# danini/multi-h

Hardware: AMD Instinct MI355X
Metric: scored homography hypotheses/sec (50k pts x 100k models) (higher is better)
Workload: dtype f64

## Files before the change

multi-h_amd/csrc/dlt4.hip:

```cpp

#include "mh_kernels.hpp"
#include "mh_device.hpp"

namespace mh {

__device__ __forceinline__ unsigned long long splitmix64(unsigned long long z)
{
    z += 0x9E3779B97F4A7C15ull;
    z = (z ^ (z >> 30)) * 0xBF58476D1CE4E5B9ull;
    z = (z ^ (z >> 27)) * 0x94D049BB133111EBull;
    return z ^ (z >> 31);
}

template <int K, int MAXDRAW>
__device__ __forceinline__ void sample_tuple(unsigned long long seed, unsigned long long m,
                                             unsigned int N, int* out)
{
    int got = 0;
    for (unsigned int c = 0; c < MAXDRAW && got < K; ++c) {
        const unsigned long long r = splitmix64(seed + (m << 8) + c);
        const int idx = (int)(((r >> 32) * (unsigned long long)N) >> 32);
        bool dup = false;
        for (int k = 0; k < got; ++k) dup = dup || (out[k] == idx);
        if (!dup) out[got++] = idx;
    }
    for (; got < K; ++got) out[got] = out[0];
}

__device__ __forceinline__ void sample4(unsigned long long seed, unsigned long long m,
                                        unsigned int N, int out[4])
{
    sample_tuple<4, 64>(seed, m, N, out);
}

constexpr int DLT_SAMPLER_UNIFORM = 0, DLT_SAMPLER_LOCAL = 1;

__device__ __forceinline__ void sample4_by(unsigned long long seed, unsigned long long c, unsigned int N, int out[4])
{
    sample4(seed, c, N, out);
}

__device__ __forceinline__ void sample4_by(unsigned long long seed, unsigned long long c, unsigned int N, int out[4],
                                           const int* __restrict__ nbr, int k, int uniform_per_16)
{
    if ((int)(c & 15ull) < uniform_per_16) { sample4(seed, c, N, out); return; }
    const unsigned long long base = seed + (c << 8);
    const int i0 = (int)(((splitmix64(base) >> 32) * (unsigned long long)N) >> 32);
    const int* __restrict__ row = nbr + (size_t)i0 * (size_t)k;
    int o1 = -1, o2 = -1, o3 = -1, got = 1;
    for (unsigned int j = 1; j < 64 && got < 4; ++j) {
        const unsigned long long r = splitmix64(base + j);
        const int cand = row[(int)(((r >> 32) * (unsigned long long)(unsigned int)k) >> 32)];
        if (cand != i0 && cand != o1 && cand != o2) {
            o1 = got == 1 ? cand : o1;
            o2 = got == 2 ? cand : o2;
            o3 = got == 3 ? cand : o3;
            ++got;
        }
    }
    out[0] = i0;
    out[1] = got > 1 ? o1 : i0;
    out[2] = got > 2 ? o2 : i0;
    out[3] = got > 3 ? o3 : i0;
}

__device__ __forceinline__ void rr_pair(int r, int slot, int& p, int& q)
{
    const int k = slot + 1;
    const int a = (r + k) % 9, b = (r + 9 - k) % 9;
    p = a < b ? a : b;
    q = a < b ? b : a;
}

constexpr int HPW = 16;
constexpr int WROWS = 17, WCOLS = 9;

__device__ __forceinline__ void wave_sync()
{
#ifdef MH_DLT_WAVE_FENCES
    __builtin_amdgcn_fence(__ATOMIC_RELEASE, "wavefront");
    __builtin_amdgcn_wave_barrier();
    __builtin_amdgcn_fence(__ATOMIC_ACQUIRE, "wavefront");
#else
    asm volatile("" ::: "memory");
    __builtin_amdgcn_wave_barrier();
    asm volatile("" ::: "memory");
#endif
}

__device__ __forceinline__ void null9_sweeps(double (*W)[HPW], int hs, int slot, bool live)
{
#define WE(r, c) W[(r) * WCOLS + (c)][hs]
    for (int sweep = 0; sweep < 30; ++sweep) {
        int rotated = 0;
        for (int r = 0; r < 9; ++r) {
            int p, q;
            rr_pair(r, slot, p, q);
            double alpha = 0.0, beta = 0.0, gamma = 0.0;
#pragma unroll
            for (int i = 0; i < 8; ++i) {
                const double wp = WE(i, p), wq = WE(i, q);
                alpha = alpha + wp * wp;
                beta = beta + wq * wq;
                gamma = gamma + wp * wq;
            }
            const bool rot = live && (gamma != 0.0) && (gamma * gamma > 1e-30 * (alpha * beta)) &&
                             (alpha >= 1e-28) && (beta >= 1e-28);
            if (rot) {
                ++rotated;
                const double zeta = (beta - alpha) / (2.0 * gamma);
                const double sg = (zeta >= 0.0) ? 1.0 : -1.0;
                const double t = sg / (fabs(zeta) + sqrt(1.0 + zeta * zeta));
                const double c = 1.0 / sqrt(1.0 + t * t);
                const double s = c * t;
#pragma unroll
                for (int i = 0; i < WROWS; ++i) {
                    const double wp = WE(i, p), wq = WE(i, q);
                    WE(i, p) = c * wp - s * wq;
                    WE(i, q) = s * wp + c * wq;
                }
            }
            wave_sync();
        }
        if (!__any(rotated)) break;
    }
#undef WE
}

__device__ __forceinline__ void null9_vector(double (*W)[HPW], int hs, double g[9])
{
#define WE(r, c) W[(r) * WCOLS + (c)][hs]
    int jm = 0;
    double best = 0.0;
    for (int j = 0; j < 9; ++j) {
        double a = 0.0;
        for (int i = 0; i < 8; ++i) a = a + WE(i, j) * WE(i, j);
        if (j == 0 || a < best) { best = a; jm = j; }
    }
    for (int j = 0; j < 9; ++j) g[j] = WE(8 + j, jm);
#undef WE
}

template <int SAMPLER, class... TABLE>
__global__ void __launch_bounds__(256) __attribute__((amdgpu_num_vgpr(72)))
k_dlt4_lds(const double* __restrict__ x1, const double* __restrict__ y1,
       const double* __restrict__ x2, const double* __restrict__ y2, int N,
       unsigned long long seed, long long first, int M, int* __restrict__ idx_out,
       double* __restrict__ H_out, TABLE... table)
{
    static_assert(sizeof...(TABLE) == (SAMPLER == DLT_SAMPLER_LOCAL ? 3 : 0), "the local sampler takes nbr, k, uniform_per_16");
    __builtin_amdgcn_s_setprio(3);
    __shared__ double sW[4][WROWS * WCOLS][HPW];
    const int lane = threadIdx.x & 63;
    const int wave = threadIdx.x >> 6;
    const int hs = lane & (HPW - 1);
    const int slot = lane >> 4;
    const int m = (blockIdx.x * 4 + wave) * HPW + hs;
    const bool live = m < M;
    double (*W)[HPW] = sW[wave];
#define WE(r, c) W[(r) * WCOLS + (c)][hs]

    int id[4] = { 0, 0, 0, 0 };
    double sx[4], sy[4], dx[4], dy[4];
    if (live) sample4_by(seed, (unsigned long long)(first + m), (unsigned int)N, id, table...);
#pragma unroll
    for (int k = 0; k < 4; ++k) {
        sx[k] = x1[id[k]]; sy[k] = y1[id[k]]; dx[k] = x2[id[k]]; dy[k] = y2[id[k]];
    }
    if (live && slot == 0 && idx_out) {
#pragma unroll
        for (int k = 0; k < 4; ++k) idx_out[4 * (size_t)m + k] = id[k];
    }
    double cx1 = ((sx[0] + sx[1]) + sx[2]) + sx[3], cy1 = ((sy[0] + sy[1]) + sy[2]) + sy[3];
    double cx2 = ((dx[0] + dx[1]) + dx[2]) + dx[3], cy2 = ((dy[0] + dy[1]) + dy[2]) + dy[3];
    cx1 = cx1 * 0.25; cy1 = cy1 * 0.25; cx2 = cx2 * 0.25; cy2 = cy2 * 0.25;
    double d1 = 0.0, d2 = 0.0;
#pragma unroll
    for (int k = 0; k < 4; ++k) {
        const double ax = sx[k] - cx1, ay = sy[k] - cy1, bx = dx[k] - cx2, by = dy[k] - cy2;
        d1 = d1 + sqrt(ax * ax + ay * ay);
        d2 = d2 + sqrt(bx * bx + by * by);
    }
    const double s1 = sqrt(2.0) / (d1 * 0.25), s2 = sqrt(2.0) / (d2 * 0.25);

    {
        double x = 0.0, y = 0.0, u = 0.0, v = 0.0;
#pragma unroll
        for (int k = 0; k < 4; ++k)
            if (k == slot) {
                x = (sx[k] - cx1) * s1; y = (sy[k] - cy1) * s1;
                u = (dx[k] - cx2) * s2; v = (dy[k] - cy2) * s2;
            }
        const int r0 = 2 * slot, r1 = 2 * slot + 1;
        WE(r0, 0) = -x; WE(r0, 1) = -y; WE(r0, 2) = -1.0; WE(r0, 3) = 0.0; WE(r0, 4) = 0.0;
        WE(r0, 5) = 0.0; WE(r0, 6) = u * x; WE(r0, 7) = u * y; WE(r0, 8) = u;
        WE(r1, 0) = 0.0; WE(r1, 1) = 0.0; WE(r1, 2) = 0.0; WE(r1, 3) = -x; WE(r1, 4) = -y;
        WE(r1, 5) = -1.0; WE(r1, 6) = v * x; WE(r1, 7) = v * y; WE(r1, 8) = v;
        if (slot < 3)
            for (int i = 3 * slot; i < 3 * slot + 3; ++i)
                for (int j = 0; j < 9; ++j) WE(8 + i, j) = (i == j) ? 1.0 : 0.0;
    }
    __syncthreads();

    null9_sweeps(W, hs, slot, live);

    if (live && slot == 0) {
        double g[9];
        null9_vector(W, hs, g);
        double A1[9];
#pragma unroll
        for (int r = 0; r < 3; ++r) {
            const double a = g[3 * r], b = g[3 * r + 1], c = g[3 * r + 2];
            A1[3 * r] = a * s1;
            A1[3 * r + 1] = b * s1;
            A1[3 * r + 2] = (c - (a * s1) * cx1) - (b * s1) * cy1;
        }
        const double is2 = 1.0 / s2;
        double Hh[9];
#pragma unroll
        for (int j = 0; j < 3; ++j) {
            Hh[j] = A1[j] * is2 + cx2 * A1[6 + j];
            Hh[3 + j] = A1[3 + j] * is2 + cy2 * A1[6 + j];
            Hh[6 + j] = A1[6 + j];
        }
        double fro = 0.0;
#pragma unroll
        for (int j = 0; j < 9; ++j) fro = fro + Hh[j] * Hh[j];
        double sc = 1.0 / sqrt(fro);
        if (Hh[8] < 0.0) sc = -sc;
        double* out = H_out + 9 * (size_t)m;
#pragma unroll
        for (int j = 0; j < 9; ++j) out[j] = Hh[j] * sc;
    }
#undef WE
}

struct Col { double v[WROWS]; };

template <int CTRL, int BANK_MASK>
__device__ __forceinline__ double dpp_merge(double old, double src)
{
    const int lo = __builtin_amdgcn_update_dpp(__double2loint(old), __double2loint(src), CTRL, 0xF, BANK_MASK, false);
    const int hi = __builtin_amdgcn_update_dpp(__double2hiint(old), __double2hiint(src), CTRL, 0xF, BANK_MASK, false);
    return __hiloint2double(hi, lo);
}

__device__ __forceinline__ void shift_columns(Col& a, Col& b, Col& c)
{
#pragma unroll
    for (int i = 0; i < WROWS; ++i) {
        c.v[i] = dpp_merge<0x114 , 0xE>(c.v[i], b.v[i]);
        b.v[i] = dpp_merge<0x104 , 0x7>(b.v[i], a.v[i]);
    }
}

__device__ __forceinline__ int rotate_pair(Col& P, Col& Q, bool swapped, bool live)
{
    double alpha = 0.0, beta = 0.0, gamma = 0.0;
#pragma unroll
    for (int i = 0; i < 8; ++i) {
        const double wp = P.v[i], wq = Q.v[i];
        alpha = alpha + wp * wp;
        beta = beta + wq * wq;
        gamma = gamma + wp * wq;
    }
    const bool rot = live && (gamma != 0.0) && (gamma * gamma > 1e-30 * (alpha * beta)) &&
                     (alpha >= 1e-28) && (beta >= 1e-28);
    if (rot) {
        const double zeta = (beta - alpha) / (2.0 * gamma);
        const bool pos = swapped ? (zeta > 0.0) : (zeta >= 0.0);
        const double sg = pos ? 1.0 : -1.0;
        const double t = sg / (fabs(zeta) + sqrt(1.0 + zeta * zeta));
        const double c = 1.0 / sqrt(1.0 + t * t);
        const double s = c * t;
#pragma unroll
        for (int i = 0; i < WROWS; ++i) {
            const double wp = P.v[i], wq = Q.v[i];
            P.v[i] = c * wp - s * wq;
            Q.v[i] = s * wp + c * wq;
        }
    }
    return rot ? 1 : 0;
}

__host__ __device__ constexpr unsigned swapped_rounds(int s)
{
    unsigned m = 0;
    for (int r = 0; r < 9; ++r) {
        const int k = s + 1, a = (r + k) % 9, b = (r + 9 - k) % 9;
        if (a > b) m |= 1u << r;
    }
    return m;
}

__device__ __forceinline__ void dlt_column(int c, const double* x, const double* y, const double* u, const double* v, Col& out)
{
#pragma unroll
    for (int k = 0; k < 4; ++k) {
        const double e0[9] = { -x[k], -y[k], -1.0, 0.0, 0.0, 0.0, u[k] * x[k], u[k] * y[k], u[k] };
        const double e1[9] = { 0.0, 0.0, 0.0, -x[k], -y[k], -1.0, v[k] * x[k], v[k] * y[k], v[k] };
        double r0 = e0[0], r1 = e1[0];
#pragma unroll
        for (int j = 1; j < 9; ++j) {
            r0 = (c == j) ? e0[j] : r0;
            r1 = (c == j) ? e1[j] : r1;
        }
        out.v[2 * k] = r0;
        out.v[2 * k + 1] = r1;
    }
#pragma unroll
    for (int i = 0; i < 9; ++i) out.v[8 + i] = (i == c) ? 1.0 : 0.0;
}

__device__ __forceinline__ double column_norm(const Col& a)
{
    double n = 0.0;
#pragma unroll
    for (int i = 0; i < 8; ++i) n = n + a.v[i] * a.v[i];
    return n;
}

template <int SAMPLER, class... TABLE>
__global__ void __launch_bounds__(256)
k_dlt4(const double* __restrict__ x1, const double* __restrict__ y1,
       const double* __restrict__ x2, const double* __restrict__ y2, int N,
       unsigned long long seed, long long first, int M, int* __restrict__ idx_out,
       double* __restrict__ H_out, TABLE... table)
{
    static_assert(sizeof...(TABLE) == (SAMPLER == DLT_SAMPLER_LOCAL ? 3 : 0), "the local sampler takes nbr, k, uniform_per_16");
    __builtin_amdgcn_s_setprio(3);
    __shared__ double sN[4][9][HPW];
    __shared__ double sK[4][6][HPW];
    const int lane = threadIdx.x & 63;
    const int wave = threadIdx.x >> 6;
    const int slot = (lane >> 2) & 3;
    const int hs = (lane >> 4) * 4 + (lane & 3);
    const int m = (blockIdx.x * 4 + wave) * HPW + hs;
    const bool live = m < M;

    Col A, B, C;
    {
        int id[4] = { 0, 0, 0, 0 };
        double sx[4], sy[4], dx[4], dy[4];
        if (live) sample4_by(seed, (unsigned long long)(first + m), (unsigned int)N, id, table...);
#pragma unroll
        for (int k = 0; k < 4; ++k) {
            sx[k] = x1[id[k]]; sy[k] = y1[id[k]]; dx[k] = x2[id[k]]; dy[k] = y2[id[k]];
        }
        if (live && slot == 0 && idx_out) {
#pragma unroll
            for (int k = 0; k < 4; ++k) idx_out[4 * (size_t)m + k] = id[k];
        }
        double cx1 = ((sx[0] + sx[1]) + sx[2]) + sx[3], cy1 = ((sy[0] + sy[1]) + sy[2]) + sy[3];
        double cx2 = ((dx[0] + dx[1]) + dx[2]) + dx[3], cy2 = ((dy[0] + dy[1]) + dy[2]) + dy[3];
        cx1 = cx1 * 0.25; cy1 = cy1 * 0.25; cx2 = cx2 * 0.25; cy2 = cy2 * 0.25;
        double d1 = 0.0, d2 = 0.0;
#pragma unroll
        for (int k = 0; k < 4; ++k) {
            const double ax = sx[k] - cx1, ay = sy[k] - cy1, bx = dx[k] - cx2, by = dy[k] - cy2;
            d1 = d1 + sqrt(ax * ax + ay * ay);
            d2 = d2 + sqrt(bx * bx + by * by);
        }
        const double s1 = sqrt(2.0) / (d1 * 0.25), s2 = sqrt(2.0) / (d2 * 0.25);
        if (slot == 0) {
            sK[wave][0][hs] = s1; sK[wave][1][hs] = s2; sK[wave][2][hs] = cx1;
            sK[wave][3][hs] = cy1; sK[wave][4][hs] = cx2; sK[wave][5][hs] = cy2;
        }
        double x[4], y[4], u[4], v[4];
#pragma unroll
        for (int k = 0; k < 4; ++k) {
            x[k] = (sx[k] - cx1) * s1; y[k] = (sy[k] - cy1) * s1;
            u[k] = (dx[k] - cx2) * s2; v[k] = (dy[k] - cy2) * s2;
        }
        dlt_column(slot + 1, x, y, u, v, A);
        dlt_column(8 - slot, x, y, u, v, B);
        dlt_column(0, x, y, u, v, C);
    }

    const unsigned sw = slot == 0 ? swapped_rounds(0) : slot == 1 ? swapped_rounds(1) : slot == 2 ? swapped_rounds(2) : swapped_rounds(3);
    for (int sweep = 0; sweep < 30; ++sweep) {
        unsigned long long rotated = 0;
#pragma unroll 1
        for (int r = 0; r < 9; r += 3) {
            rotated |= __ballot(rotate_pair(A, B, (sw >> r) & 1u, live));
            shift_columns(A, B, C);
            rotated |= __ballot(rotate_pair(B, C, (sw >> (r + 1)) & 1u, live));
            shift_columns(B, C, A);
            rotated |= __ballot(rotate_pair(C, A, (sw >> (r + 2)) & 1u, live));
            shift_columns(C, A, B);
        }
        if (rotated == 0) break;
    }

    sN[wave][slot + 1][hs] = column_norm(A);
    sN[wave][8 - slot][hs] = column_norm(B);
    if (slot == 0) sN[wave][0][hs] = column_norm(C);
    wave_sync();
    int jm = 0;
    {
        double best = 0.0;
        for (int j = 0; j < 9; ++j) {
            const double a = sN[wave][j][hs];
            if (j == 0 || a < best) { best = a; jm = j; }
        }
    }
    wave_sync();
    if (jm == slot + 1) {
#pragma unroll
        for (int j = 0; j < 9; ++j) sN[wave][j][hs] = A.v[8 + j];
    } else if (jm == 8 - slot) {
#pragma unroll
        for (int j = 0; j < 9; ++j) sN[wave][j][hs] = B.v[8 + j];
    } else if (jm == 0 && slot == 0) {
#pragma unroll
        for (int j = 0; j < 9; ++j) sN[wave][j][hs] = C.v[8 + j];
    }
    wave_sync();

    if (live && slot == 0) {
        double g[9];
#pragma unroll
        for (int j = 0; j < 9; ++j) g[j] = sN[wave][j][hs];
        const double s1 = sK[wave][0][hs], s2 = sK[wave][1][hs], cx1 = sK[wave][2][hs];
        const double cy1 = sK[wave][3][hs], cx2 = sK[wave][4][hs], cy2 = sK[wave][5][hs];
        double A1[9];
#pragma unroll
        for (int r = 0; r < 3; ++r) {
            const double a = g[3 * r], b = g[3 * r + 1], c = g[3 * r + 2];
            A1[3 * r] = a * s1;
            A1[3 * r + 1] = b * s1;
            A1[3 * r + 2] = (c - (a * s1) * cx1) - (b * s1) * cy1;
        }
        const double is2 = 1.0 / s2;
        double Hh[9];
#pragma unroll
        for (int j = 0; j < 3; ++j) {
            Hh[j] = A1[j] * is2 + cx2 * A1[6 + j];
            Hh[3 + j] = A1[3 + j] * is2 + cy2 * A1[6 + j];
            Hh[6 + j] = A1[6 + j];
        }
        double fro = 0.0;
#pragma unroll
        for (int j = 0; j < 9; ++j) fro = fro + Hh[j] * Hh[j];
        double sc = 1.0 / sqrt(fro);
        if (Hh[8] < 0.0) sc = -sc;
        double* out = H_out + 9 * (size_t)m;
#pragma unroll
        for (int j = 0; j < 9; ++j) out[j] = Hh[j] * sc;
    }
}

__global__ void __launch_bounds__(256)
k_fund8(const double* __restrict__ x1, const double* __restrict__ y1,
        const double* __restrict__ x2, const double* __restrict__ y2, int N,
        unsigned long long seed, long long first, int M, int* __restrict__ idx_out,
        double* __restrict__ F_out)
{
    __shared__ double sW[4][WROWS * WCOLS][HPW];
    const int lane = threadIdx.x & 63;
    const int wave = threadIdx.x >> 6;
    const int hs = lane & (HPW - 1);
    const int slot = lane >> 4;
    const int m = (blockIdx.x * 4 + wave) * HPW + hs;
    const bool live = m < M;
    double (*W)[HPW] = sW[wave];
#define WE(r, c) W[(r) * WCOLS + (c)][hs]

    int id[8] = { 0, 0, 0, 0, 0, 0, 0, 0 };
    if (live) sample_tuple<8, 256>(seed, (unsigned long long)(first + m), (unsigned int)N, id);
    double sx[8], sy[8], dx[8], dy[8];
#pragma unroll
    for (int k = 0; k < 8; ++k) { sx[k] = x1[id[k]]; sy[k] = y1[id[k]]; dx[k] = x2[id[k]]; dy[k] = y2[id[k]]; }
    if (live && slot == 0 && idx_out) {
#pragma unroll
        for (int k = 0; k < 8; ++k) idx_out[8 * (size_t)m + k] = id[k];
    }
    double cx1 = sx[0], cy1 = sy[0], cx2 = dx[0], cy2 = dy[0];
#pragma unroll
    for (int k = 1; k < 8; ++k) { cx1 = cx1 + sx[k]; cy1 = cy1 + sy[k]; cx2 = cx2 + dx[k]; cy2 = cy2 + dy[k]; }
    cx1 = cx1 * 0.125; cy1 = cy1 * 0.125; cx2 = cx2 * 0.125; cy2 = cy2 * 0.125;
    double d1 = 0.0, d2 = 0.0;
#pragma unroll
    for (int k = 0; k < 8; ++k) {
        const double ax = sx[k] - cx1, ay = sy[k] - cy1, bx = dx[k] - cx2, by = dy[k] - cy2;
        d1 = d1 + sqrt(ax * ax + ay * ay);
        d2 = d2 + sqrt(bx * bx + by * by);
    }
    const double s1 = sqrt(2.0) / (d1 * 0.125), s2 = sqrt(2.0) / (d2 * 0.125);

#pragma unroll
    for (int k = 0; k < 8; ++k)
        if ((k >> 1) == slot) {
            const double x = (sx[k] - cx1) * s1, y = (sy[k] - cy1) * s1;
            const double u = (dx[k] - cx2) * s2, v = (dy[k] - cy2) * s2;
            WE(k, 0) = u * x; WE(k, 1) = u * y; WE(k, 2) = u;
            WE(k, 3) = v * x; WE(k, 4) = v * y; WE(k, 5) = v;
            WE(k, 6) = x; WE(k, 7) = y; WE(k, 8) = 1.0;
        }
    if (slot < 3)
        for (int i = 3 * slot; i < 3 * slot + 3; ++i)
            for (int j = 0; j < 9; ++j) WE(8 + i, j) = (i == j) ? 1.0 : 0.0;
    __syncthreads();

    null9_sweeps(W, hs, slot, live);

    if (live && slot == 0) {
        double g[9];
        null9_vector(W, hs, g);
        double Mm[9], V[9], D[3];
        for (int i = 0; i < 3; ++i)
            for (int j = 0; j < 3; ++j) {
                double a = 0.0;
                for (int k = 0; k < 3; ++k) a = a + g[3 * k + i] * g[3 * k + j];
                Mm[3 * i + j] = a;
            }
        jacobi_sym_dev(3, Mm, V, D);
        int jm = 0;
        for (int j = 1; j < 3; ++j) if (D[j] < D[jm]) jm = j;
        const double v0 = V[0 * 3 + jm], v1 = V[1 * 3 + jm], v2 = V[2 * 3 + jm];
        double Fn[9];
        for (int r = 0; r < 3; ++r) {
            const double w = (g[3 * r] * v0 + g[3 * r + 1] * v1) + g[3 * r + 2] * v2;
            Fn[3 * r] = g[3 * r] - w * v0;
            Fn[3 * r + 1] = g[3 * r + 1] - w * v1;
            Fn[3 * r + 2] = g[3 * r + 2] - w * v2;
        }
        double B[9];
        for (int r = 0; r < 3; ++r) {
            const double a = Fn[3 * r] * s1, b = Fn[3 * r + 1] * s1;
            B[3 * r] = a; B[3 * r + 1] = b;
            B[3 * r + 2] = (Fn[3 * r + 2] - a * cx1) - b * cy1;
        }
        double Fh[9];
        const double tx = s2 * cx2, ty = s2 * cy2;
        for (int j = 0; j < 3; ++j) {
            Fh[j] = s2 * B[j];
            Fh[3 + j] = s2 * B[3 + j];
            Fh[6 + j] = (B[6 + j] - tx * B[j]) - ty * B[3 + j];
        }
        double fro = 0.0;
        for (int j = 0; j < 9; ++j) fro = fro + Fh[j] * Fh[j];
        double sc = 1.0 / sqrt(fro);
        if (Fh[8] < 0.0) sc = -sc;
        double* out = F_out + 9 * (size_t)m;
        for (int j = 0; j < 9; ++j) out[j] = Fh[j] * sc;
    }
#undef WE
}

__device__ __forceinline__ double det3_rows(const double* r0, const double* r1, const double* r2)
{
    return (r0[0] * (r1[1] * r2[2] - r1[2] * r2[1]) - r0[1] * (r1[0] * r2[2] - r1[2] * r2[0])) +
           r0[2] * (r1[0] * r2[1] - r1[1] * r2[0]);
}

__device__ __forceinline__ double cubic_newton(double c0, double c1, double c2, double c3, double t)
{
    double p = ((c3 * t + c2) * t + c1) * t + c0;
    for (int it = 0; it < 4; ++it) {
        const double dp = (3.0 * c3 * t + 2.0 * c2) * t + c1;
        const double tn = t - p / dp;
        const double pn = ((c3 * tn + c2) * tn + c1) * tn + c0;
        if (!(fabs(pn) <= fabs(p)) || !(fabs(tn) < 1e300)) break;
        t = tn; p = pn;
    }
    return t;
}

struct CubicRoots { double t0, t1, t2; int n; };

__device__ __forceinline__ CubicRoots cubic_real_roots(double c0, double c1, double c2, double c3)
{
    const double qnan = __longlong_as_double(0x7ff8000000000000ll);
    const double a = c2 / c3, b = c1 / c3, c = c0 / c3;
    const double Q = (a * a - 3.0 * b) / 9.0;
    const double R = ((2.0 * a * a * a - 9.0 * a * b) + 27.0 * c) / 54.0;
    const double Q3 = Q * Q * Q;
    const double disc = R * R - Q3;
    const double a3 = a / 3.0;
    const bool usable = (fabs(a) < 1e300) && (fabs(b) < 1e300) && (fabs(c) < 1e300) && (fabs(disc) < 1e300);
    const bool three = disc < 0.0;
    const double theta = acos(R / sqrt(Q3));
    const double sq = -2.0 * sqrt(Q);
    const double two_pi = 6.283185307179586476925286766559;
    const double u0 = sq * cos(theta / 3.0) - a3;
    const double u1 = sq * cos((theta + two_pi) / 3.0) - a3;
    const double u2 = sq * cos((theta - two_pi) / 3.0) - a3;
    double A = cbrt(fabs(R) + sqrt(disc));
    if (R >= 0.0) A = -A;
    const double B = (A == 0.0) ? 0.0 : Q / A;
    const double w0 = (A + B) - a3;
    const double w1 = -0.5 * (A + B) - a3;
    const int nr = !usable ? 0 : three ? 3 : (disc == 0.0 && Q > 0.0) ? 2 : 1;
    double r0 = nr == 0 ? qnan : cubic_newton(c0, c1, c2, c3, three ? u0 : w0);
    double r1 = nr < 2 ? qnan : cubic_newton(c0, c1, c2, c3, three ? u1 : w1);
    double r2 = nr < 3 ? qnan : cubic_newton(c0, c1, c2, c3, u2);
    { const bool sw = (r1 < r0) || (r0 != r0 && r1 == r1); const double lo = sw ? r1 : r0, hi = sw ? r0 : r1; r0 = lo; r1 = hi; }
    { const bool sw = (r2 < r1) || (r1 != r1 && r2 == r2); const double lo = sw ? r2 : r1, hi = sw ? r1 : r2; r1 = lo; r2 = hi; }
    { const bool sw = (r1 < r0) || (r0 != r0 && r1 == r1); const double lo = sw ? r1 : r0, hi = sw ? r0 : r1; r0 = lo; r1 = hi; }
    return CubicRoots{ r0, r1, r2, nr };
}

__global__ void __launch_bounds__(256)
k_fund7(const double* __restrict__ x1, const double* __restrict__ y1,
        const double* __restrict__ x2, const double* __restrict__ y2, int N,
        unsigned long long seed, long long first, int M, int* __restrict__ idx_out,
        double* __restrict__ F_out, int* __restrict__ nvalid_out)
{
    __shared__ double sW[4][WROWS * WCOLS][HPW];
    const int lane = threadIdx.x & 63;
    const int wave = threadIdx.x >> 6;
    const int hs = lane & (HPW - 1);
    const int slot = lane >> 4;
    const int m = (blockIdx.x * 4 + wave) * HPW + hs;
    const bool live = m < M;
    double (*W)[HPW] = sW[wave];
#define WE(r, c) W[(r) * WCOLS + (c)][hs]

    int id[7] = { 0, 0, 0, 0, 0, 0, 0 };
    if (live) sample_tuple<7, 256>(seed, (unsigned long long)(first + m), (unsigned int)N, id);
    double sx[7], sy[7], dx[7], dy[7];
#pragma unroll
    for (int k = 0; k < 7; ++k) { sx[k] = x1[id[k]]; sy[k] = y1[id[k]]; dx[k] = x2[id[k]]; dy[k] = y2[id[k]]; }
    if (live && slot == 0 && idx_out) {
#pragma unroll
        for (int k = 0; k < 7; ++k) idx_out[7 * (size_t)m + k] = id[k];
    }
    double cx1 = sx[0], cy1 = sy[0], cx2 = dx[0], cy2 = dy[0];
#pragma unroll
    for (int k = 1; k < 7; ++k) { cx1 = cx1 + sx[k]; cy1 = cy1 + sy[k]; cx2 = cx2 + dx[k]; cy2 = cy2 + dy[k]; }
    cx1 = cx1 / 7.0; cy1 = cy1 / 7.0; cx2 = cx2 / 7.0; cy2 = cy2 / 7.0;
    double d1 = 0.0, d2 = 0.0;
#pragma unroll
    for (int k = 0; k < 7; ++k) {
        const double ax = sx[k] - cx1, ay = sy[k] - cy1, bx = dx[k] - cx2, by = dy[k] - cy2;
        d1 = d1 + sqrt(ax * ax + ay * ay);
        d2 = d2 + sqrt(bx * bx + by * by);
    }
    const double s1 = sqrt(2.0) / (d1 / 7.0), s2 = sqrt(2.0) / (d2 / 7.0);

#pragma unroll
    for (int k = 0; k < 7; ++k)
        if ((k >> 1) == slot) {
            const double x = (sx[k] - cx1) * s1, y = (sy[k] - cy1) * s1;
            const double u = (dx[k] - cx2) * s2, v = (dy[k] - cy2) * s2;
            WE(k, 0) = u * x; WE(k, 1) = u * y; WE(k, 2) = u;
            WE(k, 3) = v * x; WE(k, 4) = v * y; WE(k, 5) = v;
            WE(k, 6) = x; WE(k, 7) = y; WE(k, 8) = 1.0;
        }
    if (slot == 3)
        for (int j = 0; j < 9; ++j) WE(7, j) = 0.0;
    if (slot < 3)
        for (int i = 3 * slot; i < 3 * slot + 3; ++i)
            for (int j = 0; j < 9; ++j) WE(8 + i, j) = (i == j) ? 1.0 : 0.0;
    __syncthreads();

    null9_sweeps(W, hs, slot, live);

    int j2 = 0, j1 = -1;
    {
        double best2 = 0.0, best1 = 0.0;
        for (int j = 0; j < 9; ++j) {
            double a = 0.0;
            for (int i = 0; i < 8; ++i) a = a + WE(i, j) * WE(i, j);
            if (j == 0 || a < best2) { best2 = a; j2 = j; }
        }
        for (int j = 0; j < 9; ++j) {
            if (j == j2) continue;
            double a = 0.0;
            for (int i = 0; i < 8; ++i) a = a + WE(i, j) * WE(i, j);
            if (j1 < 0 || a < best1) { best1 = a; j1 = j; }
        }
    }
    double G2[9], D[9];
#pragma unroll
    for (int j = 0; j < 9; ++j) { G2[j] = WE(8 + j, j2); D[j] = WE(8 + j, j1) - G2[j]; }
    const double c0 = det3_rows(G2, G2 + 3, G2 + 6);
    const double c3 = det3_rows(D, D + 3, D + 6);
    const double c1 = (det3_rows(D, G2 + 3, G2 + 6) + det3_rows(G2, D + 3, G2 + 6)) + det3_rows(G2, G2 + 3, D + 6);
    const double c2 = (det3_rows(G2, D + 3, D + 6) + det3_rows(D, G2 + 3, D + 6)) + det3_rows(D, D + 3, G2 + 6);
    const CubicRoots roots = cubic_real_roots(c0, c1, c2, c3);
    const int nroots = roots.n;

    const double t = slot == 0 ? roots.t0 : slot == 1 ? roots.t1 : roots.t2;
    double Fo[9];
    bool ok = live && slot < nroots;
    {
        double B[9];
#pragma unroll
        for (int r = 0; r < 3; ++r) {
            const double f0 = G2[3 * r] + t * D[3 * r], f1 = G2[3 * r + 1] + t * D[3 * r + 1], f2 = G2[3 * r + 2] + t * D[3 * r + 2];
            const double a = f0 * s1, b = f1 * s1;
            B[3 * r] = a; B[3 * r + 1] = b;
            B[3 * r + 2] = (f2 - a * cx1) - b * cy1;
        }
        double Fh[9];
        const double tx = s2 * cx2, ty = s2 * cy2;
#pragma unroll
        for (int j = 0; j < 3; ++j) {
            Fh[j] = s2 * B[j];
            Fh[3 + j] = s2 * B[3 + j];
            Fh[6 + j] = (B[6 + j] - tx * B[j]) - ty * B[3 + j];
        }
        double fro = 0.0;
#pragma unroll
        for (int j = 0; j < 9; ++j) fro = fro + Fh[j] * Fh[j];
        double sc = 1.0 / sqrt(fro);
        if (Fh[8] < 0.0) sc = -sc;
#pragma unroll
        for (int j = 0; j < 9; ++j) {
            Fo[j] = Fh[j] * sc;
            ok = ok && (fabs(Fo[j]) < 1e300);
        }
    }
    const unsigned long long okb = __ballot(ok);
    const int ok0 = (int)((okb >> hs) & 1ull), ok1 = (int)((okb >> (HPW + hs)) & 1ull), ok2 = (int)((okb >> (2 * HPW + hs)) & 1ull);
    const int nv = ok0 + ok1 + ok2;
    if (live && slot < 3) {
        const int place = slot == 0 ? 0 : slot == 1 ? ok0 : ok0 + ok1;
        if (ok) {
            double* out = F_out + (3 * (size_t)m + place) * 9;
#pragma unroll
            for (int j = 0; j < 9; ++j) out[j] = Fo[j];
        }
        if (slot >= nv) {
            const double qnan = __longlong_as_double(0x7ff8000000000000ll);
            double* out = F_out + (3 * (size_t)m + slot) * 9;
#pragma unroll
            for (int j = 0; j < 9; ++j) out[j] = qnan;
        }
        if (slot == 0 && nvalid_out) nvalid_out[m] = nv;
    }
#undef WE
}

hipError_t launch_fund7(const Points& p, unsigned long long seed, long long first, int M,
                        int* idx_out, double* F_out, int* nvalid_out, hipStream_t s)
{
    if (M <= 0) return hipSuccess;
    const int per_block = 4 * HPW;
    hipLaunchKernelGGL(k_fund7, dim3((M + per_block - 1) / per_block), dim3(256), 0, s, p.x1, p.y1,
                       p.x2, p.y2, p.n, seed, first, M, idx_out, F_out, nvalid_out);
    return hipGetLastError();
}

hipError_t launch_fund8(const Points& p, unsigned long long seed, long long first, int M,
                        int* idx_out, double* F_out, hipStream_t s)
{
    if (M <= 0) return hipSuccess;
    const int per_block = 4 * HPW;
    hipLaunchKernelGGL(k_fund8, dim3((M + per_block - 1) / per_block), dim3(256), 0, s, p.x1, p.y1,
                       p.x2, p.y2, p.n, seed, first, M, idx_out, F_out);
    return hipGetLastError();
}

hipError_t launch_dlt4(const Points& p, unsigned long long seed, long long first, int M,
                       int* idx_out, double* H_out, hipStream_t s, int variant, Dlt4Local local)
{
    if (M <= 0) return hipSuccess;
    const int per_block = 4 * HPW;
    const dim3 grid((M + per_block - 1) / per_block);
    if (local.nbr) {
        if (local.k < 1 || local.k >= p.n || local.uniform_per_16 < 0 || local.uniform_per_16 > 16) return hipErrorInvalidValue;
        if (variant == 1)
            hipLaunchKernelGGL((k_dlt4_lds<DLT_SAMPLER_LOCAL, const int*, int, int>), grid, dim3(256), 0, s, p.x1, p.y1,
                               p.x2, p.y2, p.n, seed, first, M, idx_out, H_out, local.nbr, local.k, local.uniform_per_16);
        else
            hipLaunchKernelGGL((k_dlt4<DLT_SAMPLER_LOCAL, const int*, int, int>), grid, dim3(256), 0, s, p.x1, p.y1,
                               p.x2, p.y2, p.n, seed, first, M, idx_out, H_out, local.nbr, local.k, local.uniform_per_16);
    } else if (variant == 1)
        hipLaunchKernelGGL(k_dlt4_lds<DLT_SAMPLER_UNIFORM>, grid, dim3(256), 0, s, p.x1, p.y1,
                           p.x2, p.y2, p.n, seed, first, M, idx_out, H_out);
    else
        hipLaunchKernelGGL(k_dlt4<DLT_SAMPLER_UNIFORM>, grid, dim3(256), 0, s, p.x1, p.y1,
                           p.x2, p.y2, p.n, seed, first, M, idx_out, H_out);
    return hipGetLastError();
}

}
```

Baseline: 13.22 million.

## Hand columns to the spare register set instead of shifting two columns per round

The one-sided Jacobi SVD's circle schedule now moves one column set per round through DPP into the spare set, where before it shifted two sets (b and c) each round. The column-to-slot mapping is tracked at compile time with a constexpr holding schedule checked by static_assert. The sweep loop is restructured into an 18-round cycle with a convergence check after each group of three, and the final column indices are recovered from the schedule phase. This roughly halves the cross-lane DPP traffic per rotation round, at the cost of more complex loop control and a re-derivation of thread indices to ease register pressure.

```diff
diff --git a/multi-h_amd/csrc/dlt4.hip b/multi-h_amd/csrc/dlt4.hip
--- a/multi-h_amd/csrc/dlt4.hip
+++ b/multi-h_amd/csrc/dlt4.hip
@@ -245,13 +245,13 @@
     return __hiloint2double(hi, lo);
 }
 
-__device__ __forceinline__ void shift_columns(Col& a, Col& b, Col& c)
-{
-#pragma unroll
-    for (int i = 0; i < WROWS; ++i) {
-        c.v[i] = dpp_merge<0x114 , 0xE>(c.v[i], b.v[i]);
-        b.v[i] = dpp_merge<0x104 , 0x7>(b.v[i], a.v[i]);
-    }
+template <bool EVEN>
+__device__ __forceinline__ void hand_on(const Col& second, Col& spare)
+{
+#pragma unroll
+    for (int i = 0; i < WROWS; ++i)
+        spare.v[i] = EVEN ? dpp_merge<0x114 , 0xE>(spare.v[i], second.v[i])
+                          : dpp_merge<0x104 , 0x7>(spare.v[i], second.v[i]);
 }
 
 __device__ __forceinline__ int rotate_pair(Col& P, Col& Q, bool swapped, bool live)
@@ -283,15 +283,58 @@
     return rot ? 1 : 0;
 }
 
+struct Holding { int col[3][4]; int first, second, spare; };
+
+__host__ __device__ constexpr Holding holding_at(int g_end)
+{
+    Holding h = { { { 2, 4, 6, 8 }, { 7, 5, 3, 1 }, { 0, -1, -1, -1 } }, 0, 1, 2 };
+    for (int g = 0; g < g_end; ++g) {
+        if (g % 2 == 0) {
+            for (int s = 3; s >= 1; --s) h.col[h.spare][s] = h.col[h.second][s - 1];
+            for (int s = 0; s < 3; ++s) h.col[h.second][s] = -1;
+        } else {
+            for (int s = 0; s < 3; ++s) h.col[h.spare][s] = h.col[h.second][s + 1];
+            for (int s = 1; s < 4; ++s) h.col[h.second][s] = -1;
+        }
+        const int f = h.first;
+        h.first = h.spare; h.spare = h.second; h.second = f;
+    }
+    return h;
+}
+
 __host__ __device__ constexpr unsigned swapped_rounds(int s)
 {
     unsigned m = 0;
-    for (int r = 0; r < 9; ++r) {
-        const int k = s + 1, a = (r + k) % 9, b = (r + 9 - k) % 9;
-        if (a > b) m |= 1u << r;
+    for (int g = 0; g < 18; ++g) {
+        const Holding h = holding_at(g);
+        if (h.col[h.first][s] > h.col[h.second][s]) m |= 1u << g;
     }
     return m;
 }
+
+__host__ __device__ constexpr bool holding_is_the_circle_schedule()
+{
+    for (int g = 0; g <= 18; ++g) {
+        const Holding h = holding_at(g);
+        const int r = g % 9;
+        if (h.first != (3 - g % 3) % 3 || h.second != (4 - g % 3) % 3) return false;
+        if (h.col[h.spare][g % 2 ? 3 : 0] != r) return false;
+        for (int k = 1; k <= 4; ++k) {
+            const int a = (r + k) % 9, b = (r + 9 - k) % 9;
+            bool found = false;
+            for (int s = 0; s < 4; ++s)
+                found = found || (h.col[h.first][s] == a && h.col[h.second][s] == b) || (h.col[h.first][s] == b && h.col[h.second][s] == a);
+            if (!found) return false;
+        }
+        if (r == 0)
+            for (int s = 0; s < 4; ++s) {
+                const int e = g == 9 ? 3 - s : s;
+                if (h.col[0][s] != 2 * e + 2 || h.col[1][s] != 7 - 2 * e) return false;
+            }
+    }
+    return true;
+}
+static_assert(holding_is_the_circle_schedule(), "k_dlt4's column hand-over does not play the circle schedule");
 
 __device__ __forceinline__ void dlt_column(int c, const double* x, const double* y, const double* u, const double* v, Col& out)
 {
@@ -319,6 +362,20 @@
     for (int i = 0; i < 8; ++i) n = n + a.v[i] * a.v[i];
     return n;
 }
+
+template <bool EVEN>
+__device__ __forceinline__ unsigned long long three_rounds(Col& A, Col& B, Col& C, unsigned sw, bool live)
+{
+    unsigned long long rotated = __ballot(rotate_pair(A, B, sw & 1u, live));
+    hand_on<EVEN>(B, C);
+    rotated |= __ballot(rotate_pair(C, A, (sw >> 1) & 1u, live));
+    hand_on<!EVEN>(A, B);
+    rotated |= __ballot(rotate_pair(B, C, (sw >> 2) & 1u, live));
+    hand_on<EVEN>(C, A);
+    return rotated;
+}
+
+__host__ __device__ constexpr int pick4(int s, const int (&t)[4]) { return s == 0 ? t[0] : s == 1 ? t[1] : s == 2 ? t[2] : t[3]; }
 
 template <int SAMPLER, class... TABLE>
 __global__ void __launch_bounds__(256)
@@ -331,14 +388,15 @@
     __builtin_amdgcn_s_setprio(3);
     __shared__ double sN[4][9][HPW];
     __shared__ double sK[4][6][HPW];
-    const int lane = threadIdx.x & 63;
-    const int wave = threadIdx.x >> 6;
-    const int slot = (lane >> 2) & 3;
-    const int hs = (lane >> 4) * 4 + (lane & 3);
-    const int m = (blockIdx.x * 4 + wave) * HPW + hs;
+    int tid = threadIdx.x;
+    int lane = tid & 63;
+    int wave = tid >> 6;
+    int slot = (lane >> 2) & 3;
+    int hs = (lane >> 4) * 4 + (lane & 3);
+    int m = (blockIdx.x * 4 + wave) * HPW + hs;
     const bool live = m < M;
-
     Col A, B, C;
+    unsigned sw;
     {
         int id[4] = { 0, 0, 0, 0 };
         double sx[4], sy[4], dx[4], dy[4];
@@ -372,29 +430,38 @@
             x[k] = (sx[k] - cx1) * s1; y[k] = (sy[k] - cy1) * s1;
             u[k] = (dx[k] - cx2) * s2; v[k] = (dy[k] - cy2) * s2;
         }
-        dlt_column(slot + 1, x, y, u, v, A);
-        dlt_column(8 - slot, x, y, u, v, B);
+        dlt_column(2 * slot + 2, x, y, u, v, A);
+        dlt_column(7 - 2 * slot, x, y, u, v, B);
         dlt_column(0, x, y, u, v, C);
-    }
-
-    const unsigned sw = slot == 0 ? swapped_rounds(0) : slot == 1 ? swapped_rounds(1) : slot == 2 ? swapped_rounds(2) : swapped_rounds(3);
-    for (int sweep = 0; sweep < 30; ++sweep) {
-        unsigned long long rotated = 0;
+        sw = slot == 0 ? swapped_rounds(0) : slot == 1 ? swapped_rounds(1) : slot == 2 ? swapped_rounds(2) : swapped_rounds(3);
+    }
+
+    int g18 = 0, thirds = 0;
+    unsigned long long rotated = 0;
+    bool go = true;
 #pragma unroll 1
-        for (int r = 0; r < 9; r += 3) {
-            rotated |= __ballot(rotate_pair(A, B, (sw >> r) & 1u, live));
-            shift_columns(A, B, C);
-            rotated |= __ballot(rotate_pair(B, C, (sw >> (r + 1)) & 1u, live));
-            shift_columns(B, C, A);
-            rotated |= __ballot(rotate_pair(C, A, (sw >> (r + 2)) & 1u, live));
-            shift_columns(C, A, B);
-        }
-        if (rotated == 0) break;
-    }
-
-    sN[wave][slot + 1][hs] = column_norm(A);
-    sN[wave][8 - slot][hs] = column_norm(B);
-    if (slot == 0) sN[wave][0][hs] = column_norm(C);
+    do {
+        rotated |= three_rounds<true>(A, B, C, sw >> g18, live);
+        ++thirds;
+        if (thirds % 3 == 0) { go = rotated != 0 && thirds < 90; rotated = 0; }
+        rotated |= three_rounds<false>(A, B, C, sw >> (g18 + 3), live && go);
+        ++thirds;
+        if (go && thirds % 3 == 0) { go = rotated != 0 && thirds < 90; rotated = 0; }
+        g18 = g18 == 12 ? 0 : g18 + 6;
+    } while (go);
+
+    asm volatile("" : "+v"(tid));
+    lane = tid & 63; wave = tid >> 6; slot = (lane >> 2) & 3; hs = (lane >> 4) * 4 + (lane & 3);
+    m = (blockIdx.x * 4 + wave) * HPW + hs;
+    constexpr Holding h0 = holding_at(0), h12 = holding_at(12);
+    static_assert(h0.first == 0 && h0.second == 1 && h12.first == 0 && h12.second == 1, "the sets play A, B, C where the loop leaves");
+    const bool whole = g18 == 0;
+    const int colA = whole ? pick4(slot, h0.col[0]) : pick4(slot, h12.col[0]);
+    const int colB = whole ? pick4(slot, h0.col[1]) : pick4(slot, h12.col[1]);
+    const int colC = whole ? h0.col[2][0] : h12.col[2][0];
+    sN[wave][colA][hs] = column_norm(A);
+    sN[wave][colB][hs] = column_norm(B);
+    if (slot == 0) sN[wave][colC][hs] = column_norm(C);
     wave_sync();
     int jm = 0;
     {
@@ -405,13 +472,13 @@
         }
     }
     wave_sync();
-    if (jm == slot + 1) {
+    if (jm == colA) {
 #pragma unroll
         for (int j = 0; j < 9; ++j) sN[wave][j][hs] = A.v[8 + j];
-    } else if (jm == 8 - slot) {
+    } else if (jm == colB) {
 #pragma unroll
         for (int j = 0; j < 9; ++j) sN[wave][j][hs] = B.v[8 + j];
-    } else if (jm == 0 && slot == 0) {
+    } else if (jm == colC && slot == 0) {
 #pragma unroll
         for (int j = 0; j < 9; ++j) sN[wave][j][hs] = C.v[8 + j];
     }
```

Result: no change. 13.25 million (median of 6 runs) (+0.2%).

## Replace two-column DPP shift with one-column hand-on Jacobi schedule and early per-round exit

Applied to the files above, without the earlier changes.

The old code moved two columns between lanes with DPP after every rotation round of the one-sided Jacobi SVD. The new code moves only one column per round, following a compile-time-checked layout that still reproduces the circle schedule over 18 rounds. It also stops as soon as nine consecutive rounds make no rotation, rather than only testing at the end of each full sweep. A lookup then finds which column each register holds when the loop ends. The aim is to roughly halve the cross-lane traffic and to cut wasted trailing rounds, at the cost of more complex bookkeeping and a slightly different rotation order that could change numerical results.

```diff
diff --git a/multi-h_amd/csrc/dlt4.hip b/multi-h_amd/csrc/dlt4.hip
--- a/multi-h_amd/csrc/dlt4.hip
+++ b/multi-h_amd/csrc/dlt4.hip
@@ -245,13 +245,96 @@
     return __hiloint2double(hi, lo);
 }
 
-__device__ __forceinline__ void shift_columns(Col& a, Col& b, Col& c)
-{
-#pragma unroll
-    for (int i = 0; i < WROWS; ++i) {
-        c.v[i] = dpp_merge<0x114 , 0xE>(c.v[i], b.v[i]);
-        b.v[i] = dpp_merge<0x104 , 0x7>(b.v[i], a.v[i]);
-    }
+template <int ODD>
+__device__ __forceinline__ void hand_on(Col& dst, const Col& src)
+{
+#pragma unroll
+    for (int i = 0; i < WROWS; ++i)
+        dst.v[i] = ODD ? dpp_merge<0x12C , 0xE>(dst.v[i], src.v[i])
+                       : dpp_merge<0x124 , 0xD>(dst.v[i], src.v[i]);
+}
+
+struct Layout { int col[4][3]; };
+
+__host__ __device__ constexpr Layout layout_start()
+{
+    return Layout{ { { 1, 8, -1 }, { 7, 2, 0 }, { 5, 4, -1 }, { 3, 6, -1 } } };
+}
+
+__host__ __device__ constexpr Layout layout_hand_on(Layout L, int r)
+{
+    const int S = r % 3, D = (r + 2) % 3, keeps = (r & 1) ? 0 : 1;
+    Layout n = L;
+    for (int s = 0; s < 4; ++s) {
+        if (s == keeps) continue;
+        const int from = (r & 1) ? (s + 1) % 4 : (s + 3) % 4;
+        n.col[s][D] = L.col[from][S];
+        n.col[from][S] = -1;
+    }
+    return n;
+}
+
+__host__ __device__ constexpr Layout layout_at(int r)
+{
+    Layout L = layout_start();
+    for (int i = 0; i < r; ++i) L = layout_hand_on(L, i);
+    return L;
+}
+
+__host__ __device__ constexpr bool schedule_ok()
+{
+    for (int r = 0; r <= 18; ++r) {
+        const Layout L = layout_at(r);
+        unsigned seen = 0;
+        for (int s = 0; s < 4; ++s) {
+            const int p = L.col[s][r % 3], q = L.col[s][(r + 1) % 3], idle = L.col[s][(r + 2) % 3];
+            if (p < 0 || q < 0 || p == q || (p + q) % 9 != (2 * r) % 9) return false;
+            if (idle >= 0 && idle != r % 9) return false;
+            seen |= (1u << p) | (1u << q) | (idle >= 0 ? 1u << idle : 0u);
+        }
+        if (seen != 0x1FFu) return false;
+        if (r == 18)
+            for (int s = 0; s < 4; ++s)
+                for (int g = 0; g < 3; ++g)
+                    if (L.col[s][g] != layout_start().col[s][g]) return false;
+    }
+    return true;
+}
+static_assert(schedule_ok(), "the one-column hand-over must re-enact the circle schedule");
+
+__host__ __device__ constexpr unsigned swapped_rounds(int s)
+{
+    unsigned m = 0;
+    for (int r = 0; r < 18; ++r) {
+        const Layout L = layout_at(r);
+        if (L.col[s][r % 3] > L.col[s][(r + 1) % 3]) m |= 1u << r;
+    }
+    return m;
+}
+
+__host__ __device__ constexpr unsigned held_places(int s, int g)
+{
+    unsigned w = 0;
+    for (int r = 0; r < 6; ++r) {
+        const int c = layout_at(r).col[s][g];
+        w |= (unsigned)(c < 0 ? 15 : (c + 9 - r) % 9) << (4 * r);
+    }
+    return w;
+}
+
+__device__ __forceinline__ unsigned by_slot(int slot, unsigned w0, unsigned w1, unsigned w2, unsigned w3)
+{
+    return slot == 0 ? w0 : slot == 1 ? w1 : slot == 2 ? w2 : w3;
+}
+
+template <int G>
+__device__ __forceinline__ int held_column(int slot, int r6, int r9)
+{
+    constexpr unsigned w0 = held_places(0, G), w1 = held_places(1, G), w2 = held_places(2, G), w3 = held_places(3, G);
+    const unsigned w = by_slot(slot, w0, w1, w2, w3);
+    const int j = (int)((w >> (4 * r6)) & 15u);
+    const int c = r9 + j;
+    return j == 15 ? -1 : (c >= 9 ? c - 9 : c);
 }
 
 __device__ __forceinline__ int rotate_pair(Col& P, Col& Q, bool swapped, bool live)
@@ -268,7 +351,7 @@
                      (alpha >= 1e-28) && (beta >= 1e-28);
     if (rot) {
         const double zeta = (beta - alpha) / (2.0 * gamma);
-        const bool pos = swapped ? (zeta > 0.0) : (zeta >= 0.0);
+        const bool pos = (zeta > 0.0) || (!swapped && zeta == 0.0);
         const double sg = pos ? 1.0 : -1.0;
         const double t = sg / (fabs(zeta) + sqrt(1.0 + zeta * zeta));
         const double c = 1.0 / sqrt(1.0 + t * t);
@@ -276,21 +359,12 @@
 #pragma unroll
         for (int i = 0; i < WROWS; ++i) {
             const double wp = P.v[i], wq = Q.v[i];
-            P.v[i] = c * wp - s * wq;
-            Q.v[i] = s * wp + c * wq;
+            const double cp = c * wp, sq = s * wq, sp = s * wp, cq = c * wq;
+            Q.v[i] = sp + cq;
+            P.v[i] = cp - sq;
         }
     }
     return rot ? 1 : 0;
-}
-
-__host__ __device__ constexpr unsigned swapped_rounds(int s)
-{
-    unsigned m = 0;
-    for (int r = 0; r < 9; ++r) {
-        const int k = s + 1, a = (r + k) % 9, b = (r + 9 - k) % 9;
-        if (a > b) m |= 1u << r;
-    }
-    return m;
 }
 
 __device__ __forceinline__ void dlt_column(int c, const double* x, const double* y, const double* u, const double* v, Col& out)
@@ -338,7 +412,7 @@
     const int m = (blockIdx.x * 4 + wave) * HPW + hs;
     const bool live = m < M;
 
-    Col A, B, C;
+    Col R0, R1, R2;
     {
         int id[4] = { 0, 0, 0, 0 };
         double sx[4], sy[4], dx[4], dy[4];
@@ -372,29 +446,47 @@
             x[k] = (sx[k] - cx1) * s1; y[k] = (sy[k] - cy1) * s1;
             u[k] = (dx[k] - cx2) * s2; v[k] = (dy[k] - cy2) * s2;
         }
-        dlt_column(slot + 1, x, y, u, v, A);
-        dlt_column(8 - slot, x, y, u, v, B);
-        dlt_column(0, x, y, u, v, C);
-    }
-
-    const unsigned sw = slot == 0 ? swapped_rounds(0) : slot == 1 ? swapped_rounds(1) : slot == 2 ? swapped_rounds(2) : swapped_rounds(3);
-    for (int sweep = 0; sweep < 30; ++sweep) {
-        unsigned long long rotated = 0;
+        constexpr Layout L0 = layout_start();
+        dlt_column((int)by_slot(slot, L0.col[0][0], L0.col[1][0], L0.col[2][0], L0.col[3][0]), x, y, u, v, R0);
+        dlt_column((int)by_slot(slot, L0.col[0][1], L0.col[1][1], L0.col[2][1], L0.col[3][1]), x, y, u, v, R1);
+        dlt_column(0, x, y, u, v, R2);
+    }
+
+    constexpr unsigned sw0 = swapped_rounds(0), sw1 = swapped_rounds(1), sw2 = swapped_rounds(2), sw3 = swapped_rounds(3);
+    const unsigned sw = by_slot(slot, sw0, sw1, sw2, sw3);
+    int rounds = 0, clean = 0, r18 = 0;
+#ifdef MH_DLT_EXIT_AT_SWEEPS
+#define MH_DLT_DONE() ((clean >= 9 && rounds % 9 == 0) || rounds == 270)
+#else
+#define MH_DLT_DONE() (clean == 9 || rounds == 270)
+#endif
+#define MH_DLT_ROUND(I, P, Q, D)                                                                   \
+    {                                                                                              \
+        const bool any = __ballot(rotate_pair(P, Q, (sw & (bit << (I))) != 0u, live)) != 0;                \
+        clean = any ? 0 : clean + 1;                                                               \
+        ++rounds;                                                                                  \
+        if (MH_DLT_DONE()) break;                                                                  \
+        hand_on<(I) & 1>(D, P);                                                                    \
+    }
 #pragma unroll 1
-        for (int r = 0; r < 9; r += 3) {
-            rotated |= __ballot(rotate_pair(A, B, (sw >> r) & 1u, live));
-            shift_columns(A, B, C);
-            rotated |= __ballot(rotate_pair(B, C, (sw >> (r + 1)) & 1u, live));
-            shift_columns(B, C, A);
-            rotated |= __ballot(rotate_pair(C, A, (sw >> (r + 2)) & 1u, live));
-            shift_columns(C, A, B);
-        }
-        if (rotated == 0) break;
-    }
-
-    sN[wave][slot + 1][hs] = column_norm(A);
-    sN[wave][8 - slot][hs] = column_norm(B);
-    if (slot == 0) sN[wave][0][hs] = column_norm(C);
+    for (;;) {
+        const unsigned bit = 1u << r18;
+        MH_DLT_ROUND(0, R0, R1, R2)
+        MH_DLT_ROUND(1, R1, R2, R0)
+        MH_DLT_ROUND(2, R2, R0, R1)
+        MH_DLT_ROUND(3, R0, R1, R2)
+        MH_DLT_ROUND(4, R1, R2, R0)
+        MH_DLT_ROUND(5, R2, R0, R1)
+        r18 = r18 == 12 ? 0 : r18 + 6;
+    }
+#undef MH_DLT_ROUND
+#undef MH_DLT_DONE
+
+    const int last = rounds - 1, r6 = last % 6, r9 = last % 9;
+    const int c0 = held_column<0>(slot, r6, r9), c1 = held_column<1>(slot, r6, r9), c2 = held_column<2>(slot, r6, r9);
+    if (c0 >= 0) sN[wave][c0][hs] = column_norm(R0);
+    if (c1 >= 0) sN[wave][c1][hs] = column_norm(R1);
+    if (c2 >= 0) sN[wave][c2][hs] = column_norm(R2);
     wave_sync();
     int jm = 0;
     {
@@ -405,15 +497,15 @@
         }
     }
     wave_sync();
-    if (jm == slot + 1) {
-#pragma unroll
-        for (int j = 0; j < 9; ++j) sN[wave][j][hs] = A.v[8 + j];
-    } else if (jm == 8 - slot) {
-#pragma unroll
-        for (int j = 0; j < 9; ++j) sN[wave][j][hs] = B.v[8 + j];
-    } else if (jm == 0 && slot == 0) {
-#pragma unroll
-        for (int j = 0; j < 9; ++j) sN[wave][j][hs] = C.v[8 + j];
+    if (jm == c0) {
+#pragma unroll
+        for (int j = 0; j < 9; ++j) sN[wave][j][hs] = R0.v[8 + j];
+    } else if (jm == c1) {
+#pragma unroll
+        for (int j = 0; j < 9; ++j) sN[wave][j][hs] = R1.v[8 + j];
+    } else if (jm == c2) {
+#pragma unroll
+        for (int j = 0; j < 9; ++j) sN[wave][j][hs] = R2.v[8 + j];
     }
     wave_sync();
 
```

After: 13.64 million before, 13.68 million after, median of 6. No clear change (+0.3%).

## Stop Jacobi SVD after nine clean rotations and use fast sqrt/rcp

Applied to the files above, without the earlier changes.

The parallel one-sided Jacobi SVD now tracks consecutive rotation steps with no active rotation and exits mid-sweep once nine clean steps pass. Before, it only checked convergence at sweep boundaries. Because the loop can now stop mid-sweep, the column-to-index mapping is tracked through r9 so norms and singular vectors are written to the correct slots. The library sqrt and division in the rotation are replaced with hardware rsq/rcp plus Newton-refinement sequences specialised for inputs in [1, ∞) and [1, √2], aimed at cutting per-rotation instruction count. The risks are bookkeeping errors in the permuted column indices and subtle rounding differences in the f64 results.

```diff
diff --git a/multi-h_amd/csrc/dlt4.hip b/multi-h_amd/csrc/dlt4.hip
--- a/multi-h_amd/csrc/dlt4.hip
+++ b/multi-h_amd/csrc/dlt4.hip
@@ -254,7 +254,32 @@
     }
 }
 
-__device__ __forceinline__ int rotate_pair(Col& P, Col& Q, bool swapped, bool live)
+__device__ __forceinline__ double sqrt_from_one(double x)
+{
+    const double y = __builtin_amdgcn_rsq(x);
+    double g = x * y, h = y * 0.5;
+    const double r = __builtin_fma(-h, g, 0.5);
+    g = __builtin_fma(g, r, g);
+    double d = __builtin_fma(-g, g, x);
+    h = __builtin_fma(h, r, h);
+    g = __builtin_fma(d, h, g);
+    d = __builtin_fma(-g, g, x);
+    g = __builtin_fma(d, h, g);
+    return __builtin_amdgcn_class(x, 0x200 ) ? x : g;
+}
+
+__device__ __forceinline__ double rcp_one_to_sqrt2(double d)
+{
+    double r = __builtin_amdgcn_rcp(d);
+    double e = __builtin_fma(-d, r, 1.0);
+    r = __builtin_fma(r, e, r);
+    e = __builtin_fma(-d, r, 1.0);
+    r = __builtin_fma(r, e, r);
+    e = __builtin_fma(-d, r, 1.0);
+    return __builtin_fma(e, r, r);
+}
+
+__device__ __forceinline__ bool rotate_pair(Col& P, Col& Q, bool swapped, bool live)
 {
     double alpha = 0.0, beta = 0.0, gamma = 0.0;
 #pragma unroll
@@ -268,19 +293,19 @@
                      (alpha >= 1e-28) && (beta >= 1e-28);
     if (rot) {
         const double zeta = (beta - alpha) / (2.0 * gamma);
-        const bool pos = swapped ? (zeta > 0.0) : (zeta >= 0.0);
-        const double sg = pos ? 1.0 : -1.0;
-        const double t = sg / (fabs(zeta) + sqrt(1.0 + zeta * zeta));
-        const double c = 1.0 / sqrt(1.0 + t * t);
+        const double sg = (zeta == 0.0) ? (swapped ? -1.0 : 1.0) : __builtin_copysign(1.0, zeta);
+        const double t = sg / (fabs(zeta) + sqrt_from_one(1.0 + zeta * zeta));
+        const double c = rcp_one_to_sqrt2(sqrt_from_one(1.0 + t * t));
         const double s = c * t;
 #pragma unroll
         for (int i = 0; i < WROWS; ++i) {
             const double wp = P.v[i], wq = Q.v[i];
-            P.v[i] = c * wp - s * wq;
-            Q.v[i] = s * wp + c * wq;
-        }
-    }
-    return rot ? 1 : 0;
+            const double sq = s * wq, sp = s * wp;
+            P.v[i] = c * wp - sq;
+            Q.v[i] = sp + c * wq;
+        }
+    }
+    return rot;
 }
 
 __host__ __device__ constexpr unsigned swapped_rounds(int s)
@@ -378,23 +403,25 @@
     }
 
     const unsigned sw = slot == 0 ? swapped_rounds(0) : slot == 1 ? swapped_rounds(1) : slot == 2 ? swapped_rounds(2) : swapped_rounds(3);
-    for (int sweep = 0; sweep < 30; ++sweep) {
-        unsigned long long rotated = 0;
+    int clean = 0;
+    int r9 = 0;
+    for (int sweep = 0; sweep < 30 && clean < 9; ++sweep) {
 #pragma unroll 1
-        for (int r = 0; r < 9; r += 3) {
-            rotated |= __ballot(rotate_pair(A, B, (sw >> r) & 1u, live));
+        for (int r = 0; r < 9 && clean < 9; r += 3) {
+            clean = __builtin_amdgcn_ballot_w64(rotate_pair(A, B, (sw >> r) & 1u, live)) ? 0 : clean + 1;
             shift_columns(A, B, C);
-            rotated |= __ballot(rotate_pair(B, C, (sw >> (r + 1)) & 1u, live));
+            if (clean < 9) clean = __builtin_amdgcn_ballot_w64(rotate_pair(B, C, (sw >> (r + 1)) & 1u, live)) ? 0 : clean + 1;
             shift_columns(B, C, A);
-            rotated |= __ballot(rotate_pair(C, A, (sw >> (r + 2)) & 1u, live));
+            if (clean < 9) clean = __builtin_amdgcn_ballot_w64(rotate_pair(C, A, (sw >> (r + 2)) & 1u, live)) ? 0 : clean + 1;
             shift_columns(C, A, B);
-        }
-        if (rotated == 0) break;
-    }
-
-    sN[wave][slot + 1][hs] = column_norm(A);
-    sN[wave][8 - slot][hs] = column_norm(B);
-    if (slot == 0) sN[wave][0][hs] = column_norm(C);
+            r9 = r == 6 ? 0 : r + 3;
+        }
+    }
+
+    const int ca = (r9 + slot + 1) % 9, cb = (r9 + 8 - slot) % 9;
+    sN[wave][ca][hs] = column_norm(A);
+    sN[wave][cb][hs] = column_norm(B);
+    if (slot == 0) sN[wave][r9][hs] = column_norm(C);
     wave_sync();
     int jm = 0;
     {
@@ -405,13 +432,13 @@
         }
     }
     wave_sync();
-    if (jm == slot + 1) {
+    if (jm == ca) {
 #pragma unroll
         for (int j = 0; j < 9; ++j) sN[wave][j][hs] = A.v[8 + j];
-    } else if (jm == 8 - slot) {
+    } else if (jm == cb) {
 #pragma unroll
         for (int j = 0; j < 9; ++j) sN[wave][j][hs] = B.v[8 + j];
-    } else if (jm == 0 && slot == 0) {
+    } else if (jm == r9 && slot == 0) {
 #pragma unroll
         for (int j = 0; j < 9; ++j) sN[wave][j][hs] = C.v[8 + j];
     }
```

Result: no change. 13.68 million before, 13.73 million after, median of 6 (+0.3%).
